# csiro-robotics/syropod_highlevel_controller

Measured on AMD Instinct MI355X. Metric: control-cycles/sec (all legs IK-solved), higher is better.
Workload: dtype f64

## Files before the change

syropod_highlevel_controller_amd/csrc/shc_cycle_kernel.hpp:

```cpp
#pragma once

#include "shc_cycle.hpp"
#include "shc_cycle_launch.hpp"

#include <hip/hip_runtime.h>

namespace shc {

#ifndef SHC_WAVES_PER_SIMD
#define SHC_WAVES_PER_SIMD 2
#endif
#ifndef SHC_ROT_WAVES_PER_SIMD
#define SHC_ROT_WAVES_PER_SIMD 1
#endif
#ifndef SHC_TERRAIN_WAVES_PER_SIMD
#define SHC_TERRAIN_WAVES_PER_SIMD 2
#endif

struct LegPlanes {
  double2 *base;
  int64_t ns;
  uint32_t slot;
  typedef double v2d __attribute__((ext_vector_type(2)));
  __device__ __forceinline__ double2 load(int plane) const { return (base + plane * ns)[slot]; }
// ... 442 lines not shown
        const double fn = norm(in.force());
        const double defined = ld_agent_f64(sp2 + 1);
        if (fn > A.touchdown_threshold && defined == 0.0) {
          Chain<NJ> ch;
          fk_chain<NJ>(C.leg[leg], s.q, ch);
          const V3 tipnow = tip_robot_frame(C.leg[leg], ch.pe);
          if (live) sp[0] = tipnow.x, sp[1] = tipnow.y, sp2[0] = tipnow.z, sp2[1] = 1.0;
        } else if (fn < A.liftoff_threshold) {
          if (live) sp2[1] = 0.0;
        }
      }
    }
    cycle<L, NJ, F>(s, out, C, rb, pk, g, leg, st.legd, ns, slot, dirty, manual_live, touchdown_detection, ext, nullptr, in, publish_previous,
                    (F & F_ROUGH) != 0 ? st.span : nullptr);
    {
      typedef unsigned v4u __attribute__((ext_vector_type(4)));
      double flat[2 * NJ];
#pragma unroll
      for (int i = 0; i < NJ; ++i) flat[FD::Q + i] = s.q[i], flat[FD::QD + i] = s.qd[i];
      const unsigned soff = oslot * out_slot_bytes;
      if (live) {
#pragma unroll
        for (int p = 0; p < NJ; ++p) {
          const u64 a = u64(__double_as_longlong(flat[2 * p])), b = u64(__double_as_longlong(flat[2 * p + 1]));
          const v4u w = {unsigned(a), unsigned(a >> 32), unsigned(b), unsigned(b >> 32)};
          __builtin_amdgcn_raw_buffer_store_b128(w, out_rsrc, unsigned((int64_t(p) * ns + slot) * 16), soff, 16 );
        }
      }
    }
    ++c;
    oslot = oslot + 1 == unsigned(A.depth) ? 0 : oslot + 1;
    gate = uni64(gate_next_v);
    hdr_valid = next_valid;
    if (next_valid) h0 = uni64(n0v), h1 = uni64(n1v);
  }
  if constexpr (!batch) {
    asm volatile("s_waitcnt vmcnt(0)" ::: "memory");
    if (lane == 0) st_agent(A.progress + wave, u64(c));
  }
  held.cycles = c;
}

template <int L, int NJ>
__device__ __forceinline__ void carry_leg_inputs(const ResidentArgs &A, const DevState &st, const ResidentHeld &held, const int64_t ns, const uint32_t slot, const int leg) {
  using FD = Fields<NJ>;
  constexpr int RPW = 64 / L;
  double2 *planes = reinterpret_cast<double2 *>(st.legd);
  const LegInRing<NJ> in = leg_inputs_in_force<L, NJ>(A, st.legd, held.src_force, held.src_effort, ns, slot, int64_t(slot / 64) * RPW + (slot % 64) / L, leg,
                                                      A.batch_cycles ? int64_t(A.batch_cycles) - 1 : 0);
  if (held.src_force != -1) {
    const V3 f = in.force();
    planes[(FD::FORCE_IN / 2) * ns + slot] = double2{f.x, f.y};
    planes[(FD::FORCE_IN / 2 + 1) * ns + slot] = double2{f.z, 0.0};
  }
  if (held.src_effort != -1) {
    double ef[NJ];
    in.effort(ef);
#pragma unroll
    for (int p = 0; p < FD::NJE / 2; ++p) planes[(FD::EFFORT_IN / 2 + p) * ns + slot] = double2{ef[2 * p], 2 * p + 1 < NJ ? ef[2 * p + 1] : 0.0};
  }
}

template <int L, int NJ, unsigned F>
__device__ __forceinline__ void resident_epilogue(const ResidentArgs &A, const DevState &st, const uint32_t slot, const int lane, const bool live,
                                                  const double *tile, const int32_t *tile_i, double *gtile, int32_t *gtile_i, const ResidentHeld &held) {
  using R = RobotFields;
  using FD = Fields<NJ>;
  constexpr int RPW = 64 / L;
  const int64_t ns = st.n_slots;
  store_rob_fields<RPW, R::VIN, R::CORE_END>(tile, gtile, lane);
  if (held.seen & (1u << RG_IMU)) {
    store_rob_fields<RPW, R::GYRO, R::IMU_END>(tile, gtile, lane);
    store_rob_fields<RPW, R::IMUQ, R::IMUQ_END>(tile, gtile, lane);
  }
  if ((held.seen & (1u << RG_RESET)) && lane < RPW) gtile_i[R::I_RESET_MODE * RPW + lane] = tile_i[R::I_RESET_MODE * RPW + lane];
  if (live) carry_leg_inputs<L, NJ>(A, st, held, ns, slot, int(slot % 64) % L);
  if (lane == 0 && A.batch_cycles == 0) {
    if (held.fault) __hip_atomic_fetch_or(&A.ctl->fault, 1ull, __ATOMIC_RELAXED, __HIP_MEMORY_SCOPE_AGENT);
    __hip_atomic_fetch_add(&A.ctl->exited, 1ull, __ATOMIC_RELAXED, __HIP_MEMORY_SCOPE_AGENT);
  }
}

enum : int { PART_BOTH = 0, PART_GATE = 1, PART_DONE = 2 };
template <int PART>
__device__ __forceinline__ void resident_relay(const ResidentArgs &A) {
  const int lane = threadIdx.x & 63;
  const unsigned max_cycles = A.max_cycles;
  unsigned db = 0, sp = max_cycles, idle_stop = 0xffffffffu;
  u64 reason = RESIDENT_EXIT_MAX, last_reason = 0, last_gate = ~0ull, last_done = 0, iter = 0;
  u64 t_last = wall_clock64(), t_all_done = 0;
  for (;;) {
    const u64 now = wall_clock64();
    const u64 exited_v = ld_agent(&A.ctl->exited);
    const u64 gate_v = PART == PART_DONE ? ld_agent(&A.ctl->gate) : 0;
    const u64 done_v = PART != PART_DONE ? ld_agent(&A.ctl->pad[1]) : 0;
    u64 pv[8];
    if (PART != PART_GATE) {
#pragma unroll
      for (int j = 0; j < 8; ++j) pv[j] = j * 64 + lane < A.n_waves ? ld_agent(A.progress + j * 64 + lane) : ~0ull;
    }
    if (PART != PART_DONE) {
      const u64 hd_v = ld_sys(&A.host->doorbell), hs_v = ld_sys(&A.host->stop);
      const u64 rec_v = lane < 2 ? ld_sys(&A.host->records[size_t(db & (kResidentHeaders - 1)) * 2 + lane]) : 0;
      const u64 hd = uni64(hd_v), hs = uni64(hs_v);
      unsigned want_db = hd > max_cycles ? max_cycles : unsigned(hd);
      if (want_db < db) want_db = db;
      if (want_db == db && db < max_cycles) {
        const u64 tag = u64(db) + 1;
        const bool word_ok = lane == 0 ? rec_v == tag : (lane == 1 ? (rec_v >> 48) == (tag & 0xffffull) : true);
        if (__all(word_ok)) {
          const u64 w1 = uni64(__shfl(rec_v, 1, 64));
          if (lane == 0) {
            u64 *hp = reinterpret_cast<u64 *>(A.headers + (db & (kResidentHeaders - 1)));
            st_agent(hp + 1, (w1 & 0x7fffull) | u64(kResidentDirect) | (w1 & 0x30000ull));
            st_agent(hp, tag);
          }
          asm volatile("s_waitcnt vmcnt(0)" ::: "memory");
          want_db = db + 1;
        }
      }
      if (want_db != db || uni64(done_v) < u64(db)) t_last = now;
      else if (idle_stop == 0xffffffffu && now - t_last > A.idle_ticks) idle_stop = db;
      unsigned want_sp = max_cycles;
      u64 why = RESIDENT_EXIT_MAX;
      if (hs <= max_cycles) want_sp = unsigned(hs), why = RESIDENT_EXIT_STOP;
      if (idle_stop < want_sp) want_sp = idle_stop, why = RESIDENT_EXIT_IDLE;
      if (want_sp < db) want_sp = db;
      if (want_db > want_sp) want_db = want_sp;
      db = want_db, sp = want_sp, reason = why;
      if (reason != last_reason) {
        if (lane == 0) st_agent(&A.ctl->pad[0], reason);
        last_reason = reason;
      }
      const u64 gate = (u64(sp) << 32) | db;
      if (gate != last_gate) {
        if (lane == 0) st_agent(&A.ctl->gate, gate);
        last_gate = gate;
      }
    }
    const u64 exited = uni64(exited_v);
    bool leave = exited == u64(A.n_waves);
    if (PART != PART_GATE) {
      if (PART == PART_DONE) sp = unsigned(uni64(gate_v) >> 32);
      u64 m = ~0ull;
#pragma unroll
      for (int j = 0; j < 8; ++j) m = pv[j] < m ? pv[j] : m;
      for (int64_t base = 512; base < A.n_waves; base += 512) {
        u64 v[8];
#pragma unroll
        for (int j = 0; j < 8; ++j) {
          const int64_t w = base + j * 64 + lane;
          v[j] = w < A.n_waves ? ld_agent(A.progress + w) : ~0ull;
        }
#pragma unroll
        for (int j = 0; j < 8; ++j) m = v[j] < m ? v[j] : m;
      }
#pragma unroll
      for (int off = 32; off > 0; off >>= 1) {
        const u64 o = __shfl_xor(m, off, 64);
        m = o < m ? o : m;
      }
      m = uni64(m);
      if (m != last_done) {
        if (lane == 0) {
          st_sys(&A.host->done, m);
          st_agent(&A.ctl->pad[1], m);
        }
        last_done = m;
      }
      bool gave_up = false;
      if (!leave && m >= sp) {
        if (t_all_done == 0) t_all_done = now;
        else if (now - t_all_done > 5000 * A.ticks_per_ms) leave = gave_up = true;
      }
      if (leave) {
        const u64 fault = uni64(ld_agent(&A.ctl->fault));
        const u64 why = uni64(ld_agent(&A.ctl->pad[0]));
        if (lane == 0) {
          st_sys(&A.host->fault, fault);
          st_sys(&A.host->done, m);
          st_agent(&A.ctl->pad[1], m);
          asm volatile("s_waitcnt vmcnt(0)" ::: "memory");
          st_agent(&A.ctl->pad[2], 1ull);
          st_sys(&A.host->exited, (fault || gave_up) ? u64(RESIDENT_EXIT_FAULT) : why);
        }
      }
      if ((++iter & 1023) == 0 && lane == 0) st_sys(&A.host->heartbeat, iter);
    }
    if (leave) break;
    __builtin_amdgcn_s_sleep(1);
  }
}

template <int L, int NJ, unsigned F, bool RES, int HALF = ROLE_ALL, bool BATCH = false>
__device__ __forceinline__ void cycle_wave(const DevState &st, const SharedConsts<L, NJ> *gc, int n_cycles, unsigned rt_flags, const int64_t wave,
                                           const ResidentArgs *ra) {
  static_assert(HALF == ROLE_ALL || (!RES && (F & (F_DYN | F_TERRAIN | F_MLEGS | F_AUTO)) == 0), "half-step launches: feature-exact kernels without auto posing / terrain paths");
  using R = RobotFields;
  using FT = Feat<F>;
  constexpr int RPW = 64 / L;
  __shared__ SharedConsts<L, NJ> C;
  extern __shared__ double wave_lds[];
  constexpr int kWaveDoubles = R::COUNT * RPW + PK_COUNT * 64 + (R::I_COUNT * RPW + 1) / 2;
  SHC_TICK(0);
  const bool manual_live = (rt_flags & RT_MANUAL_LIVE) != 0;
  const bool touchdown_detection = (rt_flags & RT_TOUCHDOWN) != 0;
  const int lane = threadIdx.x & 63;
  const int wib = threadIdx.x >> 6;
  const int64_t rob0 = wave * RPW;
  const int64_t left = st.n_robots - rob0;
  const int robots_here = left < RPW ? (left < 0 ? 0 : int(left)) : RPW;
  int grp = lane / L;
  const int leg = lane - grp * L;
  const bool live = grp < robots_here;
  if (grp >= robots_here) grp = robots_here > 0 ? robots_here - 1 : 0;
  const uint32_t slot = uint32_t(wave * 64 + grp * L + leg);
  double *const my_lds = wave_lds + wib * kWaveDoubles;
  Park pk{my_lds + R::COUNT * RPW, lane};
  LegRegs<NJ> s;
  const CycleParams &GP = gc->P;
  double *tile = my_lds;
  int32_t *tile_i = reinterpret_cast<int32_t *>(my_lds + R::COUNT * RPW + PK_COUNT * 64);
  double *gtile = st.robd + wave * (R::COUNT * RPW);
  int32_t *gtile_i = st.robi + wave * (R::I_COUNT * RPW);
  LegLoad<NJ> ll;
  double th[NJ];
  const bool any_robot = robots_here > 0;
  double2 hand[4] = {double2{0.0, 0.0}, double2{0.0, 0.0}, double2{0.0, 0.0}, double2{0.0, 0.0}};
  double hpose[7] = {0.0, 0.0, 0.0, 1.0, 0.0, 0.0, 0.0};
  double2 qpl[(NJ + 1) / 2];
  int word_back = 0;
  if (any_robot) {
#pragma unroll
    for (int k = 0; k < NJ; ++k) th[k] = gc->leg[leg].link_th[k];
    load_leg_issue<NJ, F, HALF>(ll, st, GP, slot);
    if constexpr (HALF == ROLE_FRONT) {
#pragma unroll
      for (int p = 0; p < (NJ + 1) / 2; ++p) qpl[p] = reinterpret_cast<const double2 *>(st.legd)[p * st.n_slots + slot];
    }
    if constexpr (HALF == ROLE_BACK) {
      word_back = st.legi[slot];
      using FDh = Fields<NJ>;
      static_assert(FDh::TIP % 2 == 0 && FDh::CUR_DIR == FDh::ORG_DIR + 3 && FDh::ORG_DIR % 2 == 0, "plane layout of the walker tip / tip direction");
      const double2 *planes = reinterpret_cast<const double2 *>(st.legd);
      hand[0] = planes[(FDh::TIP / 2) * st.n_slots + slot];
      hand[1] = planes[(FDh::TIP / 2 + 1) * st.n_slots + slot];
      hand[2] = planes[(FDh::ORG_DIR / 2 + 1) * st.n_slots + slot];
      hand[3] = planes[(FDh::ORG_DIR / 2 + 2) * st.n_slots + slot];
#pragma unroll
      for (int k = 0; k < 7; ++k) hpose[k] = gtile[(R::CPOSE + k) * RPW + grp];
    }
  }
  using SC = SharedConsts<L, NJ>;
  static_assert(sizeof(SC) % 16 == 0 && (offsetof(SC, P) + offsetof(CycleParams, ap_start)) % 16 == 0, "const block is copied in 16-byte words");
  constexpr int n16_all = sizeof(SC) / 16;
  constexpr int n16_core = (offsetof(SC, P) + offsetof(CycleParams, ap_start)) / 16;
  const int n16 = FT::autop(GP) ? n16_all : n16_core;
  constexpr int citers = (n16_all + 63) / 64;
  double2 creg[citers];
  {
    const double2 *src = reinterpret_cast<const double2 *>(gc);
    const int nt = blockDim.x;
#pragma unroll
    for (int it = 0; it < citers; ++it) {
      int i = it * nt + threadIdx.x;
      creg[it] = i < n16 ? src[i] : double2{0.0, 0.0};
    }
  }
  double t_core[(R::CORE_END * RPW + 63) / 64], t_man[((R::MANUAL_END - R::MPOSE) * RPW + 63) / 64],
      t_imu[((R::IMU_END - R::ABSE) * RPW + 63) / 64], t_imuq[((R::IMUQ_END - R::IMUQ) * RPW + 63) / 64],
      t_aprev[((R::APREV_END - R::APREV) * RPW + 63) / 64], t_align[((R::COUNT - R::TALIGN) * RPW + 63) / 64], t_odom[((R::ODOM_END - R::ODOM) * RPW + 63) / 64],
      t_cpose[((R::CPOSE_END - R::CPOSE) * RPW + 63) / 64], t_incl[((R::INCL_END - R::INCL) * RPW + 63) / 64];
  const bool skip_marked = (F & F_MLEGS) != 0 && (rt_flags & RT_SKIP_MARKED) != 0 && (rt_flags & RT_MANUAL_LEGS) != 0;
  const bool pose_marked = (F & F_MLEGS) != 0 && (rt_flags & RT_POSE_MARKED) != 0 && (rt_flags & RT_MANUAL_LEGS) != 0;
// ... 274 lines not shown
  if (POSE_SPLIT && walker && lane == 0) X.pose_done[pair] = 0;
  __syncthreads();
  const CycleParams &P = C.P;
  Group<L> g{grp * L};
  RobTile<RPW> rb{tile, tile_i, grp};
  LegOut out;
  out.poser_tip = out.model_tip = out.adm_delta = V3{0, 0, 0};
  s.tipx = V3{1, 0, 0};
  if (active && !walker) {
#pragma unroll
    for (int k = 0; k < NJ; ++k) sincos_joint(C.leg[leg].link_th[k] + s.q[k], &s.sn[k], &s.cs[k]);
    if (FT::adm(P) || LegRegs<NJ>::kKeepJacobian) {
      Chain<NJ> ch;
      chain_from_sincos<NJ>(C.leg[leg], s.sn, s.cs, ch);
      if (LegRegs<NJ>::kKeepJacobian) {
        jacobian_columns<NJ>(ch, s.lin);
        s.pe = ch.pe;
      }
      if (FT::adm(P)) s.tipx = base_rotate(C.leg[leg], ch.xe);
    }
    s.word = 0;
  }
  unsigned dirty = 0;
  ResidentHeld held;
  const int swing_c_count_u = uni(P.swing_c_count);
  const auto publish_for_pose = [&](unsigned cycle, bool planes) {
    if (planes) {
      const V3 pp = rb.get3(R::PLANE_PREV), pn = rb.get3(R::PNORM_PREV);
#pragma unroll
      for (int par = 0; par < 2; ++par) {
        double *mb = &X.mailbox[pair][par][0][lane];
        mb[7 * 64] = pp.x, mb[8 * 64] = pp.y, mb[9 * 64] = pp.z, mb[10 * 64] = pn.x, mb[11 * 64] = pn.y, mb[12 * 64] = pn.z;
      }
    }
    X.pose_c[pair][cycle & 1][lane] = walk_plane_control_candidate<L, NJ>(s.word, C, P, swing_c_count_u);
  };
  if (POSE_SPLIT && walker && active) publish_for_pose(0, true);
  const int64_t ns = st.n_slots;
  const unsigned out_slot_bytes = unsigned(NJ * ns * 16);
  const __amdgpu_buffer_rsrc_t out_rsrc = __builtin_amdgcn_make_buffer_rsrc(A.out, 0, int(unsigned(A.depth) * out_slot_bytes), 0x00020000);
  const u64 emergency_ticks = 4 * A.idle_ticks + 2000 * A.ticks_per_ms;
  unsigned k = 0, c_front = 0, c_back = 0, oslot = 0;
  bool prev_real = false;
  u64 prev_h0 = 0, prev_h1 = 0;
  u64 gate_pref = leader ? ld_agent(&A.ctl->gate) : 0;
  u64 bubble_since = 0;
  FrontToBack fb{V3{1, 0, 0}, false, LS_WALKING};
  fb.uf = load_uni_flags(C.P);
  OdomCache odom_cache;
  Pose owpp_cache = pose_identity();
  if (POSE_SPLIT && active && !walker) owpp_cache = rb.getpose(R::OWPP);
  constexpr bool ODOM_REGS = NJ <= 3;
  constexpr bool ODOM_WALKER = NJ > 3 || (F & (F_ADM | F_IMU | F_INCL | F_AUTO | F_DYN)) != 0;
  double odom[4] = {0.0, 0.0, 1.0, 0.0};
  if (ODOM_REGS && FT::odom(P) && active && walker == ODOM_WALKER) {
#pragma unroll
    for (int i = 0; i < 4; ++i) odom[i] = rb.get(R::ODOM + i);
  }
#ifdef SHC_RES2_TIMING
  long long tm_busy = 0, tm_total0 = __builtin_readcyclecounter(), tm_real = 0;
#ifndef SHC_RES2_BUSY_ONLY
  if (threadIdx.x < 64) shc_acc_lds[threadIdx.x] = 0;
#endif
#endif
#ifdef SHC_RES2_TIMING
#define SHC_R2_ITER_BEGIN() const long long tm0 = __builtin_readcyclecounter(); SHC_TICK(19)
#ifndef SHC_RES2_BUSY_ONLY
#define SHC_R2_PHASES(THREAD, ...)                                                                                                  \
  if (kind == IT_REAL && prev_real && blockIdx.x == 1 && threadIdx.x == (THREAD)) {       \
    const int base = ((THREAD) >> 7) * 32;                                                                                         \
    const int order[] = {__VA_ARGS__};                                                                                             \
    for (int i = 1; i < int(sizeof(order) / sizeof(int)); ++i) shc_acc_lds[base + order[i]] += shc_ticks_lds[base + order[i]] - shc_ticks_lds[base + order[i - 1]]; \
  }
#else
#define SHC_R2_PHASES(THREAD, ...)
#endif
#define SHC_R2_ITER_END(THREAD, ...)                                                         \
  if (kind == IT_REAL && prev_real) tm_busy += __builtin_readcyclecounter() - tm0, ++tm_real; \
  SHC_R2_PHASES(THREAD, __VA_ARGS__)
#else
#define SHC_R2_ITER_BEGIN() do {} while (0)
#define SHC_R2_ITER_END(THREAD, ...) do {} while (0)
#endif
  LegInRing<NJ> in_at;
  int in_src_force = -1000, in_src_effort = -1000;
  if (walker) {
    for (;;) {
      SHC_R2_ITER_BEGIN();
      const int kind = __builtin_amdgcn_readfirstlane(int(X.ctrl[k & 3][0]));
      const u64 h0 = uni64(X.ctrl[k & 3][1]), h1 = uni64(X.ctrl[k & 3][2]);
      SHC_TICK(20);
      if (kind == IT_REAL && active) {
        resident_take_inputs<RPW, POSE_SPLIT ? ROBOT_VEL : ROBOT_ALL, false>(A, c_front, h0, h1, wave, lane, tile, tile_i, dirty, held, st.n_robots);
        SHC_TICK(21);
        const PoseWait<RPW> pose_wait{&X.pose_done[pair], c_front + 1, A.ticks_per_ms, &held.fault};
        cycle_front<L, NJ, F, false, LegInRing<NJ>, false, !POSE_SPLIT>(s, out, C, rb, pk, g, leg, st.legd, ns, slot, dirty, manual_live, false, nullptr, nullptr,
                                                                        LegInRing<NJ>{}, fb, nullptr, pose_wait);
#ifdef SHC_ABLATE
        if (!(P.debug_skip & 65536))
#endif
        if (POSE_SPLIT) publish_for_pose(c_front + 1, fb.plane_prev_changed);
        SHC_TICK(29);
        double *mb = &X.mailbox[pair][c_front & 1][0][lane];
        mb[0] = out.poser_tip.x, mb[64] = out.poser_tip.y, mb[128] = out.poser_tip.z;
        if constexpr (ODOM_WALKER) {
          if (FT::odom(P) && __any(fb.odom_run)) {
            if (fb.odom_run) {
              if constexpr (ODOM_REGS) odometry_advance(odom[0], odom[1], odom[2], odom[3], P, fb.odom_vel.x, fb.odom_vel.y, fb.odom_vel.z, &odom_cache);
              else odometry_step(rb, P, fb.odom_vel.x, fb.odom_vel.y, fb.odom_vel.z, &odom_cache);
            }
          }
        } else if (FT::odom(P)) {
          mb[192] = fb.odom_vel.x, mb[256] = fb.odom_vel.y, mb[320] = fb.odom_vel.z, mb[384] = fb.odom_run ? 1.0 : 0.0;
        }
        SHC_TICK(22);
      }
      SHC_TICK(23);
      if (kind == IT_EXIT) break;
      SHC_R2_ITER_END(0, 19, 20, 21, 2, 3, 4, 5, 6, 7, 16, 8, 17, 15, 29, 22, 23);
      if (kind == IT_REAL) ++c_front;
      prev_real = kind == IT_REAL;
      __syncthreads();
      ++k;
    }
  } else {
    for (;;) {
      SHC_R2_ITER_BEGIN();
      const int kind = __builtin_amdgcn_readfirstlane(int(X.ctrl[k & 3][0]));
      const u64 h0 = uni64(X.ctrl[k & 3][1]), h1 = uni64(X.ctrl[k & 3][2]);
      SHC_TICK(29);
      int nk = IT_EXIT;
      u64 nh0v = 0, nh1v = 0;
      if (leader && kind != IT_EXIT) {
        u64 gate;
        if (kind == IT_BUBBLE) {
          __builtin_amdgcn_s_sleep(2);
          gate = uni64(ld_agent(&A.ctl->gate));
        } else {
          gate = uni64(gate_pref);
        }
        const unsigned db = unsigned(gate), sp = unsigned(gate >> 32);
        const unsigned cn = c_front + (kind == IT_REAL ? 1u : 0u);
        nk = cn >= sp ? IT_EXIT : (cn < db ? IT_REAL : IT_BUBBLE);
        if (nk == IT_BUBBLE) {
          const u64 now = wall_clock64();
          if (bubble_since == 0) bubble_since = now;
          else if (now - bubble_since > emergency_ticks) nk = IT_EXIT, held.fault = true;
        } else {
          bubble_since = 0;
        }
        if (nk == IT_REAL) {
          const u64 *hp = reinterpret_cast<const u64 *>(A.headers + (cn & (kResidentHeaders - 1)));
          nh0v = ld_agent(hp);
          nh1v = ld_agent(hp + 1);
        }
        if (kind == IT_BUBBLE) gate_pref = gate;
        else gate_pref = ld_agent(&A.ctl->gate);
      }
      if (active) {
        SHC_TICK(24);
        if constexpr (POSE_SPLIT) if (kind == IT_REAL) {
          resident_take_inputs<RPW, ROBOT_POSE, false>(A, c_front, h0, h1, wave, lane, tile, tile_i, dirty, held, st.n_robots);
          SHC_TICK(30);
          double pose_c = -1.0;
#pragma unroll
          for (int j = 0; j < L; ++j) {
            const double cj = X.pose_c[pair][c_front & 1][g.base + j];
            pose_c = cj >= 0.0 ? cj : pose_c;
          }
          int lw[L] = {};
          const double *mb = &X.mailbox[pair][c_front & 1][0][lane];
          const V3 plane_prev{mb[7 * 64], mb[8 * 64], mb[9 * 64]}, pnorm_prev{mb[10 * 64], mb[11 * 64], mb[12 * 64]};
          int rword_unused = 0;
          Pose ap = pose_identity(), la = pose_identity();
#ifdef SHC_ABLATE
          if (!(P.debug_skip & 2048))
#endif
          (void)cycle_pose<L, NJ, F, true>(s, C, P, C.leg[leg], rb, g, leg, lw, rword_unused, 0, dirty, manual_live, ap, la, plane_prev, pnorm_prev, fb.uf.swing_c_count, 0,
                                           &owpp_cache, &pose_c);
          __builtin_amdgcn_fence(__ATOMIC_RELEASE, "workgroup");
          __builtin_amdgcn_wave_barrier();
          if (lane == 0) *const_cast<volatile unsigned *>(&X.pose_done[pair]) = c_front + 1;
        }
        SHC_TICK(25);
        if (prev_real) {
          resident_take_inputs<RPW, ROBOT_NONE, true>(A, c_back, prev_h0, prev_h1, wave, lane, tile, tile_i, dirty, held, st.n_robots);
          if (held.src_force != in_src_force || held.src_effort != in_src_effort) {
            in_at = leg_inputs_in_force<L, NJ>(A, st.legd, held.src_force, held.src_effort, ns, slot, wave * RPW + grp, leg);
            in_src_force = held.src_force, in_src_effort = held.src_effort;
          }
          LegInRing<NJ> in = in_at;
          if (FT::tipf(P)) in.prefetch_effort();
          SHC_TICK(31);
          const double *mb = &X.mailbox[pair][c_back & 1][0][lane];
          out.poser_tip = V3{mb[0], mb[64], mb[128]};
          if constexpr (!ODOM_WALKER) if (FT::odom(P)) {
            const V3 ov{mb[192], mb[256], mb[320]};
            if (__any(mb[384] != 0.0)) {
              if (mb[384] != 0.0) {
                if constexpr (ODOM_REGS) odometry_advance(odom[0], odom[1], odom[2], odom[3], P, ov.x, ov.y, ov.z, &odom_cache);
                else odometry_step(rb, P, ov.x, ov.y, ov.z, &odom_cache);
              }
            }
          }
          out.adm_delta = V3{0, 0, 0};
          if (FT::adm(P)) cycle_admittance<NJ>(s, out, P, in);
          s.word = 0;
          SHC_TICK(26);
          cycle_back<L, NJ, F>(s, out, C, leg, st.legd, ns, slot, nullptr, in, fb);
          SHC_TICK(27);
          asm volatile("s_waitcnt vmcnt(0)" ::: "memory");
          if (lane == 0) st_agent(A.progress + wave, u64(c_back));
          SHC_TICK(13);
          {
            typedef unsigned v4u __attribute__((ext_vector_type(4)));
            double flat[2 * NJ];
#pragma unroll
            for (int i = 0; i < NJ; ++i) flat[FD::Q + i] = s.q[i], flat[FD::QD + i] = s.qd[i];
            const unsigned soff = oslot * out_slot_bytes;
#ifdef SHC_ABLATE
            if (!(P.debug_skip & 4096))
#endif
            if (live) {
#pragma unroll
              for (int p = 0; p < NJ; ++p) {
                const u64 a = u64(__double_as_longlong(flat[2 * p])), b = u64(__double_as_longlong(flat[2 * p + 1]));
                const v4u w = {unsigned(a), unsigned(a >> 32), unsigned(b), unsigned(b >> 32)};
                __builtin_amdgcn_raw_buffer_store_b128(w, out_rsrc, unsigned((int64_t(p) * ns + slot) * 16), soff, 16 );
              }
            }
          }
          ++c_back;
          oslot = oslot + 1 == unsigned(A.depth) ? 0 : oslot + 1;
          SHC_TICK(28);
        }
        if (kind != IT_REAL) {
          asm volatile("s_waitcnt vmcnt(0)" ::: "memory");
          if (lane == 0) st_agent(A.progress + wave, u64(c_back));
        }
      }
      if (leader && kind != IT_EXIT && lane == 0) {
        X.ctrl[(k + 1) & 3][0] = u64(nk);
        X.ctrl[(k + 1) & 3][1] = nh0v;
        X.ctrl[(k + 1) & 3][2] = nh1v;
      }
      SHC_TICK(14);
      if (kind == IT_EXIT) break;
      SHC_R2_ITER_END(128, 19, 29, 24, 30, 25, 31, 26, 9, 10, 11, 12, 27, 13, 28, 14);
      if (kind == IT_REAL) ++c_front;
      prev_real = kind == IT_REAL;
      prev_h0 = h0, prev_h1 = h1;
      __syncthreads();
      ++k;
    }
  }
#undef SHC_R2_ITER_BEGIN
#undef SHC_R2_ITER_END
#undef SHC_R2_PHASES
#ifdef SHC_RES2_TIMING
  if (blockIdx.x == 1 && lane == 0 && pair == 0) {
    unsigned long long *dbg = reinterpret_cast<unsigned long long *>(A.ctl) + 8 + (walker ? 0 : 4);
    dbg[0] = tm_busy, dbg[1] = tm_real, dbg[2] = __builtin_readcyclecounter() - tm_total0, dbg[3] = k;
#ifndef SHC_RES2_BUSY_ONLY
    if (walker) {
      for (int i = 0; i < 32; ++i) dbg[8 + i] = (unsigned long long)shc_acc_lds[i];
    } else {
      for (int i = 0; i < 32; ++i) dbg[36 + i] = (unsigned long long)shc_acc_lds[32 + i];
    }
#endif
  }
#endif
  if (active && ODOM_REGS && FT::odom(P) && walker == ODOM_WALKER) {
#pragma unroll
    for (int i = 0; i < 4; ++i) rb.put(R::ODOM + i, odom[i]);
  }
  if (active) {
    if (walker) {
      X.stiff[pair][lane] = s.stiff;
    } else {
      X.ikfail[pair][lane] = s.word & LW_IKFAIL;
      if (POSE_SPLIT) {
        unsigned d = 0;
#pragma unroll
        for (unsigned b = 1; b <= DIRTY_LAST; b <<= 1)
          if (__any((dirty & b) != 0)) d |= b;
        if (lane == 0) X.model_dirty[pair] = d, X.model_seen[pair] = held.seen;
      }
      if (lane == 0) X.model_fault[pair] = held.fault ? 1u : 0u;
    }
  }
  __syncthreads();
  if (!active) return;
  if (walker) {
    if (POSE_SPLIT) dirty |= X.model_dirty[pair], held.seen |= X.model_seen[pair];
    if (X.model_fault[pair]) held.fault = true;
    if (c_front > 0) s.word = (s.word & ~LW_IKFAIL) | X.ikfail[pair][lane];
    {
      unsigned d = 0;
#pragma unroll
      for (unsigned b = 1; b <= DIRTY_LAST; b <<= 1)
        if (__any((dirty & b) != 0)) d |= b;
      dirty = d;
    }
    if (live) store_leg<NJ, F, ROLE_FRONT>(s, out, pk, st, P, slot, dirty);
    __builtin_amdgcn_wave_barrier();
    store_rob_fields<RPW, 0, R::PLANE>(tile, gtile, lane);
    if (dirty & DIRTY_WALK_PLANE) store_rob_fields<RPW, R::PLANE, R::VIN>(tile, gtile, lane);
    if (FT::manual(P) && manual_live && (dirty & DIRTY_MANUAL)) store_rob_fields<RPW, R::MPOSE, R::MANUAL_END>(tile, gtile, lane);
    if (FT::imu(P)) store_rob_fields<RPW, R::ABSE, R::GYRO>(tile, gtile, lane);
    if (FT::incl(P) && FT::autop(P)) store_rob_fields<RPW, R::APREV, R::APREV_END>(tile, gtile, lane);
    store_rob_fields<RPW, R::CPOSE, R::CPOSE_END>(tile, gtile, lane);
    if (FT::odom(P)) store_rob_fields<RPW, R::ODOM, R::ODOM_END>(tile, gtile, lane);
    if (lane < (R::I_POSE_PHASE + 1) * RPW) gtile_i[lane] = tile_i[lane];
    store_rob_fields<RPW, R::VIN, R::CORE_END>(tile, gtile, lane);
    if (held.seen & (1u << RG_IMU)) {
      store_rob_fields<RPW, R::GYRO, R::IMU_END>(tile, gtile, lane);
      store_rob_fields<RPW, R::IMUQ, R::IMUQ_END>(tile, gtile, lane);
    }
    if ((held.seen & (1u << RG_RESET)) && lane < RPW) gtile_i[R::I_RESET_MODE * RPW + lane] = tile_i[R::I_RESET_MODE * RPW + lane];
    if (lane == 0) {
      if (held.fault) __hip_atomic_fetch_or(&A.ctl->fault, 1ull, __ATOMIC_RELAXED, __HIP_MEMORY_SCOPE_AGENT);
      __hip_atomic_fetch_add(&A.ctl->exited, 1ull, __ATOMIC_RELAXED, __HIP_MEMORY_SCOPE_AGENT);
    }
  } else {
    s.stiff = X.stiff[pair][lane];
    if (live) {
      store_leg<NJ, F, ROLE_BACK>(s, out, pk, st, P, slot, 0);
      carry_leg_inputs<L, NJ>(A, st, held, ns, slot, leg);
    }
  }
}

}
```

syropod_highlevel_controller_amd/csrc/shc_resident.hpp:

```cpp

struct Resident {
  bool active = false;
  int depth = 0;
  ResidentArgs args{};
  ResidentHost *host = nullptr;
  ResidentHost *host_dev = nullptr;
  ResidentCtl *ctl = nullptr;
  unsigned long long *progress = nullptr;
  ResidentHeader *headers = nullptr;
  double *rin = nullptr, *force = nullptr, *effort = nullptr, *out = nullptr, *stage = nullptr;
  int32_t *rini = nullptr;
  size_t stage_bytes = 0;
  static constexpr int kPinSlots = 4;
  unsigned *post_blocks_done = nullptr;
  char *pin = nullptr, *pin_dev = nullptr;
  hipEvent_t pin_ev[kPinSlots] = {};
  unsigned long long pin_uses = 0;
  hipStream_t in_stream = nullptr;
  hipStream_t loop_stream = nullptr;
  hipEvent_t loop_ev = nullptr;
  unsigned long long published = 0;
  unsigned long long posted = 0;
  unsigned long long posts[RG_COUNT] = {};
  std::vector<unsigned long long> post_cycle[RG_COUNT];
// ... 519 lines not shown
}

extern "C" int shc_engine_resident_get_joint_state_async(shc_engine *e, int64_t cycle, double *q, double *qd, int timeout_ms) {
  int rc = resident_require(e, true);
  if (rc != SHC_OK) return rc;
  Resident *r = e->res;
  if ((rc = resident_alive(r)) != SHC_OK) return rc;
  if (cycle < 0 || (unsigned long long)cycle >= r->max_cycles) return fail(SHC_ERR_INVALID_ARG, "resident mode: no such cycle (max_cycles)");
  if (r->published > (unsigned long long)cycle + r->depth)
    return fail(SHC_ERR_INVALID_ARG, "resident mode: that cycle's outputs may have been overwritten (ring_depth newer cycles were published)");
  HIP_TRY(hipSetDevice(e->device));
  const unsigned long long ticks = (unsigned long long)(timeout_ms > 0 ? timeout_ms : 5000) * r->wall_khz;
  resident_wait_done_kernel<<<dim3(1), dim3(1), 0, e->stream>>>(r->ctl, r->host_dev, (unsigned long long)cycle + 1, ticks);
  HIP_TRY(hipGetLastError());
  const double *slot = r->out + size_t(cycle % r->depth) * size_t(e->NJ) * e->n_slots * 2;
  const int64_t threads = e->n * e->L;
  for (int which = 0; which < 2; ++which) {
    double *dst = which ? qd : q;
    if (!dst) continue;
    gather_leg_kernel<<<dim3((unsigned)((threads + 63) / 64)), dim3(64), 0, e->stream>>>(dst, slot, e->n_slots, e->n, e->L, e->NJ,
                                                                                         which ? LEG_FIELD(e, QD) : LEG_FIELD(e, Q));
    HIP_TRY(hipGetLastError());
  }
  return SHC_OK;
}

extern "C" int shc_engine_resident_status(shc_engine *e, int64_t *published, int64_t *completed, int32_t *running) {
  int rc = resident_require(e, false);
  if (rc != SHC_OK) return rc;
  Resident *r = e->res;
  const bool active = r && r->active;
  if (published) *published = active ? int64_t(r->published) : 0;
  if (completed) *completed = active ? int64_t(host_load(&r->host->done)) : 0;
  if (running) *running = active && host_load(&r->host->exited) == 0 ? 1 : 0;
  return SHC_OK;
}

extern "C" int shc_engine_resident_end(shc_engine *e, int64_t *cycles_run) {
  int rc = resident_require(e, true);
  if (rc != SHC_OK) return rc;
  Resident *r = e->res;
  HIP_TRY(hipSetDevice(e->device));
  HIP_TRY(hipStreamSynchronize(r->in_stream));
  const int direct_rc = resident_wait_direct_installed(r);
  const std::string direct_msg = direct_rc != SHC_OK ? std::string(shc_last_error()) : std::string();
  if (direct_rc == SHC_OK) host_store(&r->host->doorbell, r->published);
  host_store(&r->host->stop, direct_rc == SHC_OK ? r->published : 0ull);
  const bool answered = spin_until([&] { return host_load(&r->host->exited) != 0; }, r->poisoned ? 5.0 : 30.0);
  if (!answered) {
    r->poisoned = true;
    return fail(SHC_ERR_TIMEOUT, "resident mode: the device loop did not answer the stop request in time; the engine stays in resident mode - call "
                                 "shc_engine_resident_end again");
  }
  hipError_t err = hipStreamSynchronize(r->loop_stream);
  if (err == hipSuccess) err = hipStreamSynchronize(e->stream);
  r->active = false;
  r->poisoned = false;
#ifdef SHC_RES2_TIMING
  if (err == hipSuccess) {
    ResidentCtl c;
    (void)hipMemcpy(&c, r->ctl, sizeof c, hipMemcpyDeviceToHost);
    for (int w = 0; w < 2; ++w)
      fprintf(stderr, "[res2 timing] %s: %.0f clocks busy per steady REAL iteration (%llu of them), loop %llu clocks, %llu iterations\n", w ? "model " : "walker",
              c.dbg[4 * w + 1] ? double(c.dbg[4 * w]) / double(c.dbg[4 * w + 1]) : 0.0, c.dbg[4 * w + 1], c.dbg[4 * w + 2], c.dbg[4 * w + 3]);
#ifndef SHC_RES2_BUSY_ONLY
    const int order[] = {20, 21, 2, 3, 4, 5, 6, 7, 16, 8, 17, 15, 29, 22, 23};
    const char *wname[] = {"control words (LDS) read", "inputs of the cycle taken", "cycle_front entry", "robot word / command read, stop predicates", "(pose elsewhere)", "getLimit",
                           "velocity shaping", "walk state machine", "stepper (stride, Bezier, tip)", "tip rotation / iteratePhase / planes / leg word", "wait for the pose flag",
                           "pose read + updateStance", "control input for the next pose published", "mailbox written", "to the barrier"};
    const double its = c.dbg[1] ? double(c.dbg[1]) : 1.0;
    fprintf(stderr, "[res2 timing] walker of pair 0, mean clocks per phase:\n");
    for (int i = 0; i < int(sizeof(order) / sizeof(int)); ++i) fprintf(stderr, "[res2 timing]   walker t%-2d %-58s %7.0f\n", order[i], wname[i], double(c.dbg[8 + order[i]]) / its);
    const int morder[] = {29, 24, 30, 25, 31, 26, 9, 10, 11, 12, 27, 13, 28, 14};
    const char *mname[] = {"control words (LDS) read", "leader: gate, what the next iteration is, header prefetch issued", "pose inputs of the cycle taken",
                           "updateCurrentPose of the walker's cycle + flag", "leg inputs in force, joint efforts prefetched", "mailbox read, odometry, admittance",
                           "cycle_back entry (desired tip)", "IK step + joint update", "sin / cos, chain, Jacobian", "model tip, tip force", "cycle_back exit",
                           "wait for the previous stores + progress word", "output-ring stores issued", "control words written (leader: waits for its loads)"};
    const double mits = c.dbg[5] ? double(c.dbg[5]) : 1.0;
    fprintf(stderr, "[res2 timing] model wavefront of pair 0 (the leader), mean clocks per phase:\n");
    for (int i = 0; i < int(sizeof(morder) / sizeof(int)); ++i) fprintf(stderr, "[res2 timing]   model  t%-2d %-58s %7.0f\n", morder[i], mname[i], double(c.dbg[40 + morder[i]]) / mits);
#endif
  }
#endif
  const unsigned long long reason = host_load(&r->host->exited), done = host_load(&r->host->done);
  if (cycles_run) *cycles_run = int64_t(done);
  if (r->groups_posted & (1u << RG_FORCE)) e->rt_flags |= RT_TOUCHDOWN;
  if (err != hipSuccess) return fail(SHC_ERR_HIP, std::string("hipStreamSynchronize: ") + hipGetErrorString(err));
  if (direct_rc != SHC_OK) return fail(direct_rc, direct_msg + " (the loop was stopped after " + std::to_string(done) + " cycles)");
  if (reason == RESIDENT_EXIT_FAULT || host_load(&r->host->fault) != 0)
    return fail(SHC_ERR_HIP, "resident mode: a wavefront gave up waiting for the relay; restore the engine from a snapshot");
  if (host_load(&r->host->late_reads) != 0)
    return fail(SHC_ERR_TIMEOUT, "resident mode: a stream-ordered read (shc_engine_resident_get_joint_state_async) gave up waiting for its cycle");
  if (!((reason == RESIDENT_EXIT_STOP || reason == RESIDENT_EXIT_MAX) && done == r->published))
    return fail(SHC_ERR_TIMEOUT, std::string("resident mode: the device loop had stopped by itself (") +
                                     (reason == RESIDENT_EXIT_IDLE ? "idle timeout" : reason == RESIDENT_EXIT_MAX ? "max_cycles" : "unknown") + ") after " +
                                     std::to_string(done) + " of " + std::to_string(r->published) + " published cycles");
  return SHC_OK;
}

static int step_k_out_ring(shc_engine *e, int K) {
  const size_t need = size_t(K) * size_t(e->NJ) * size_t(e->n_slots) * 16;
  if (e->k_out && e->k_out_bytes >= need) return SHC_OK;
  if (e->k_out) {
    const int rc = join_side(e);
    if (rc != SHC_OK) return rc;
    HIP_TRY(hipStreamSynchronize(e->stream));
    (void)hipFree(e->k_out);
    e->k_out = nullptr, e->k_out_bytes = 0;
  }
  HIP_TRY(hipMalloc(reinterpret_cast<void **>(&e->k_out), need));
  e->k_out_bytes = need;
  return SHC_OK;
}

__global__ void copy_joint_planes_kernel(double2 *dst, const double2 *src, int64_t count);
static int step_k_serial(shc_engine *e, int K, const shc_cycle_inputs *in) {
  const int64_t n = e->n, slot = int64_t(e->NJ) * e->n_slots;
  for (int k = 0; k < K; ++k) {
    int rc = SHC_OK;
    if (in && in->linear_xy) rc = shc_engine_set_velocity(e, in->linear_xy + k * n * 2, in->angular + k * n, 1);
    if (rc == SHC_OK && in && in->imu_orientation_wxyz) rc = shc_engine_set_imu(e, in->imu_orientation_wxyz + k * n * 4, in->imu_angular_velocity + k * n * 3, 1);
    if (rc == SHC_OK && in && in->tip_force) rc = shc_engine_set_tip_force(e, in->tip_force + k * n * e->L * 3, 1);
    if (rc == SHC_OK && in && in->joint_effort) rc = shc_engine_set_joint_effort(e, in->joint_effort + k * n * e->L * e->NJ, 1);
    if (rc == SHC_OK) rc = shc_engine_step(e, 1);
    if (rc == SHC_OK) rc = join_side(e);
    if (rc != SHC_OK) return rc;
    copy_joint_planes_kernel<<<dim3((unsigned)((slot + 255) / 256)), dim3(256), 0, e->stream>>>(reinterpret_cast<double2 *>(e->k_out) + k * slot,
                                                                                              reinterpret_cast<const double2 *>(e->st.legd), slot);
    HIP_TRY(hipGetLastError());
  }
  e->k_out_cycles = K;
  return SHC_OK;
}

extern "C" int shc_engine_step_k(shc_engine *e, int n_cycles, const shc_cycle_inputs *in) {
  SHC_ENTER(e);
  if (n_cycles < 1 || n_cycles > 4096) return fail(SHC_ERR_INVALID_ARG, "shc_engine_step_k: 1 .. 4096 cycles per launch");
  if (e->starting_up) return fail(SHC_ERR_UNSUPPORTED, "shc_engine_step_k starts from a running engine (finish the start-up first)");
  unsigned mask = 0;
  if (in) {
    if (!in->on_device) return fail(SHC_ERR_INVALID_ARG, "shc_engine_step_k: the K-deep input arrays are device arrays (on_device = 1)");
    if ((in->linear_xy == nullptr) != (in->angular == nullptr)) return fail(SHC_ERR_INVALID_ARG, "linear_xy and angular are given together");
    if ((in->imu_orientation_wxyz == nullptr) != (in->imu_angular_velocity == nullptr)) return fail(SHC_ERR_INVALID_ARG, "the two IMU arrays are given together");
    if (in->pose_translation_velocity || in->pose_rotation_velocity || in->pose_reset_mode)
      return fail(SHC_ERR_UNSUPPORTED, "shc_engine_step_k carries velocity, IMU, tip force and joint effort; give pose inputs / reset modes with their setters before the call (held for the K cycles)");
    if (in->linear_xy) mask |= 1u << RG_VEL;
    if (in->imu_orientation_wxyz) mask |= 1u << RG_IMU;
    if (in->tip_force) mask |= 1u << RG_FORCE;
    if (in->joint_effort) mask |= 1u << RG_EFFORT;
  }
  HIP_TRY(hipSetDevice(e->device));
  const bool split = e->n_waves >= kSplitWaves && !(e->features & SHC_FEAT_SINGLE_STREAM);
  if (!split || ((mask & (1u << RG_EFFORT)) && !(e->rt_flags & RT_EFFORT_LIVE))) {
    const int rc = join_side(e);
    if (rc != SHC_OK) return rc;
  }
  if (mask & (1u << RG_EFFORT)) {
    const int rc = effort_live(e);
    if (rc != SHC_OK) return rc;
  }
  ResidentFit fit;
  {
    const int rc = resident_fit(e, fit);
    if (rc != SHC_OK) return rc;
  }
  if (size_t(e->NJ) * e->n_slots * 16 * size_t(n_cycles) >= (size_t(1) << 31))
// ... 80 lines not shown
```

Baseline: 1.573 billion.

## Pipeline relay doorbell polling with multiple in-flight samples and drop gate sleep

The gate-side relay now keeps several doorbell/control samples in flight in a small ring, processing one sample while the next loads are outstanding, and no longer sleeps between polls. Each sample's host and control words are gathered by lane and read with readlane. The done-side progress scan uses wider unrolled batches, and model wavefronts reuse a prefetched gate value when a bubble is followed by another non-real iteration. The aim is to cut host-doorbell-to-device latency in the resident loop, at the cost of acting on slightly stale samples and busier polling of system memory.

```diff
diff --git a/syropod_highlevel_controller_amd/csrc/shc_cycle_kernel.hpp b/syropod_highlevel_controller_amd/csrc/shc_cycle_kernel.hpp
--- a/syropod_highlevel_controller_amd/csrc/shc_cycle_kernel.hpp
+++ b/syropod_highlevel_controller_amd/csrc/shc_cycle_kernel.hpp
@@ -548,114 +548,162 @@
 }
 
 enum : int { PART_BOTH = 0, PART_GATE = 1, PART_DONE = 2 };
+#ifndef SHC_RELAY_DEPTH
+#define SHC_RELAY_DEPTH 4
+#endif
+static_assert(SHC_RELAY_DEPTH >= 1 && SHC_RELAY_DEPTH <= 4, "doorbell samples in flight");
+#ifndef SHC_DONE_ROUND
+#define SHC_DONE_ROUND 16
+#endif
+struct RelaySample {
+  u64 host_v;
+  u64 ctl_v;
+  unsigned db;
+};
+static_assert(offsetof(ResidentCtl, dbg) == 64 && offsetof(ResidentHost, doorbell) == 0 && offsetof(ResidentHost, stop) == 8 && offsetof(ResidentCtl, gate) == 0 && offsetof(ResidentCtl, exited) == 8 && offsetof(ResidentCtl, pad) == 24, "the samples address these words by lane");
+__device__ __forceinline__ RelaySample relay_sample_issue(const ResidentArgs &A, const unsigned db, const int lane) {
+  const int l4 = lane & 3;
+  const u64 *hp = l4 < 2 ? reinterpret_cast<const u64 *>(A.host) + l4 : &A.host->records[size_t(db & (kResidentHeaders - 1)) * 2 + (l4 & 1)];
+  return RelaySample{ld_sys(hp), ld_agent(reinterpret_cast<const u64 *>(A.ctl) + (lane & 7)), db};
+}
+__device__ __forceinline__ u64 lane64(const u64 v, const int l) {
+  return (u64(unsigned(__builtin_amdgcn_readlane(int(unsigned(v >> 32)), l))) << 32) | unsigned(__builtin_amdgcn_readlane(int(unsigned(v)), l));
+}
 template <int PART>
 __device__ __forceinline__ void resident_relay(const ResidentArgs &A) {
+  constexpr int D = PART == PART_GATE ? SHC_RELAY_DEPTH : 1;
   const int lane = threadIdx.x & 63;
   const unsigned max_cycles = A.max_cycles;
   unsigned db = 0, sp = max_cycles, idle_stop = 0xffffffffu;
   u64 reason = RESIDENT_EXIT_MAX, last_reason = 0, last_gate = ~0ull, last_done = 0, iter = 0;
   u64 t_last = wall_clock64(), t_all_done = 0;
+#ifdef SHC_RELAY_TIMING
+  const u64 tm_begin = wall_clock64();
+#endif
+  RelaySample ring[D];
+  if (PART != PART_DONE) {
+#pragma unroll
+    for (int i = 0; i < D; ++i) ring[i] = relay_sample_issue(A, db, lane);
+  }
+  bool leave = false;
   for (;;) {
-    const u64 now = wall_clock64();
-    const u64 exited_v = ld_agent(&A.ctl->exited);
-    const u64 gate_v = PART == PART_DONE ? ld_agent(&A.ctl->gate) : 0;
-    const u64 done_v = PART != PART_DONE ? ld_agent(&A.ctl->pad[1]) : 0;
-    u64 pv[8];
-    if (PART != PART_GATE) {
-#pragma unroll
-      for (int j = 0; j < 8; ++j) pv[j] = j * 64 + lane < A.n_waves ? ld_agent(A.progress + j * 64 + lane) : ~0ull;
-    }
-    if (PART != PART_DONE) {
-      const u64 hd_v = ld_sys(&A.host->doorbell), hs_v = ld_sys(&A.host->stop);
-      const u64 rec_v = lane < 2 ? ld_sys(&A.host->records[size_t(db & (kResidentHeaders - 1)) * 2 + lane]) : 0;
-      const u64 hd = uni64(hd_v), hs = uni64(hs_v);
-      unsigned want_db = hd > max_cycles ? max_cycles : unsigned(hd);
-      if (want_db < db) want_db = db;
-      if (want_db == db && db < max_cycles) {
-        const u64 tag = u64(db) + 1;
-        const bool word_ok = lane == 0 ? rec_v == tag : (lane == 1 ? (rec_v >> 48) == (tag & 0xffffull) : true);
-        if (__all(word_ok)) {
-          const u64 w1 = uni64(__shfl(rec_v, 1, 64));
+#pragma unroll
+    for (int i = 0; i < D; ++i) {
+      const u64 now = wall_clock64();
+      u64 exited = 0;
+      bool posted = false;
+      if (PART != PART_DONE) {
+        const RelaySample s = ring[i];
+        const u64 hd = lane64(s.host_v, 0), hs = lane64(s.host_v, 1);
+        const u64 done_v = lane64(s.ctl_v, 4);
+        exited = lane64(s.ctl_v, 1);
+        unsigned want_db = hd > max_cycles ? max_cycles : unsigned(hd);
+        if (want_db < db) want_db = db;
+        if (want_db == db && db < max_cycles && s.db == db) {
+          const u64 tag = u64(db) + 1;
+          const bool word_ok = lane == 2 ? s.host_v == tag : (lane == 3 ? (s.host_v >> 48) == (tag & 0xffffull) : true);
+          if (__all(word_ok)) {
+            const u64 w1 = lane64(s.host_v, 3);
+            if (lane == 0) {
+              u64 *hp = reinterpret_cast<u64 *>(A.headers + (db & (kResidentHeaders - 1)));
+              st_agent(hp + 1, (w1 & 0x7fffull) | u64(kResidentDirect) | (w1 & 0x30000ull));
+              st_agent(hp, tag);
+            }
+            posted = true;
+            want_db = db + 1;
+          }
+        }
+        if (want_db != db || done_v < u64(db)) t_last = now;
+        else if (idle_stop == 0xffffffffu && now - t_last > A.idle_ticks) idle_stop = db;
+        unsigned want_sp = max_cycles;
+        u64 why = RESIDENT_EXIT_MAX;
+        if (hs <= max_cycles) want_sp = unsigned(hs), why = RESIDENT_EXIT_STOP;
+        if (idle_stop < want_sp) want_sp = idle_stop, why = RESIDENT_EXIT_IDLE;
+        if (want_sp < db) want_sp = db;
+        if (want_db > want_sp) want_db = want_sp;
+        db = want_db, sp = want_sp, reason = why;
+      }
+      u64 ctl_now = 0, pv[SHC_DONE_ROUND];
+      if (PART == PART_DONE) ctl_now = lane < 2 ? ld_agent(reinterpret_cast<const u64 *>(A.ctl) + lane) : 0;
+      if (PART != PART_GATE) {
+#pragma unroll
+        for (int j = 0; j < SHC_DONE_ROUND; ++j) pv[j] = j * 64 + lane < A.n_waves ? ld_agent(A.progress + j * 64 + lane) : ~0ull;
+      }
+      if (PART != PART_DONE) {
+        ring[i] = relay_sample_issue(A, db, lane);
+        if (posted) asm volatile("s_waitcnt vmcnt(0)" ::: "memory");
+        if (reason != last_reason) {
+          if (lane == 0) st_agent(&A.ctl->pad[0], reason);
+          last_reason = reason;
+        }
+        const u64 gate = (u64(sp) << 32) | db;
+        if (gate != last_gate) {
+          if (lane == 0) st_agent(&A.ctl->gate, gate);
+          last_gate = gate;
+        }
+      }
+      if (PART == PART_DONE) exited = lane64(ctl_now, 1);
+      leave |= exited == u64(A.n_waves);
+      if (PART != PART_GATE) {
+        if (PART == PART_DONE) sp = unsigned(lane64(ctl_now, 0) >> 32);
+        u64 m = ~0ull;
+#pragma unroll
+        for (int j = 0; j < SHC_DONE_ROUND; ++j) m = pv[j] < m ? pv[j] : m;
+        for (int64_t base = 64 * SHC_DONE_ROUND; base < A.n_waves; base += 64 * SHC_DONE_ROUND) {
+          u64 v[SHC_DONE_ROUND];
+#pragma unroll
+          for (int j = 0; j < SHC_DONE_ROUND; ++j) {
+            const int64_t w = base + j * 64 + lane;
+            v[j] = w < A.n_waves ? ld_agent(A.progress + w) : ~0ull;
+          }
+#pragma unroll
+          for (int j = 0; j < SHC_DONE_ROUND; ++j) m = v[j] < m ? v[j] : m;
+        }
+#pragma unroll
+        for (int off = 32; off > 0; off >>= 1) {
+          const u64 o = __shfl_xor(m, off, 64);
+          m = o < m ? o : m;
+        }
+        m = uni64(m);
+        if (m != last_done) {
           if (lane == 0) {
-            u64 *hp = reinterpret_cast<u64 *>(A.headers + (db & (kResidentHeaders - 1)));
-            st_agent(hp + 1, (w1 & 0x7fffull) | u64(kResidentDirect) | (w1 & 0x30000ull));
-            st_agent(hp, tag);
+            st_sys(&A.host->done, m);
+            st_agent(&A.ctl->pad[1], m);
           }
-          asm volatile("s_waitcnt vmcnt(0)" ::: "memory");
-          want_db = db + 1;
-        }
-      }
-      if (want_db != db || uni64(done_v) < u64(db)) t_last = now;
-      else if (idle_stop == 0xffffffffu && now - t_last > A.idle_ticks) idle_stop = db;
-      unsigned want_sp = max_cycles;
-      u64 why = RESIDENT_EXIT_MAX;
-      if (hs <= max_cycles) want_sp = unsigned(hs), why = RESIDENT_EXIT_STOP;
-      if (idle_stop < want_sp) want_sp = idle_stop, why = RESIDENT_EXIT_IDLE;
-      if (want_sp < db) want_sp = db;
-      if (want_db > want_sp) want_db = want_sp;
-      db = want_db, sp = want_sp, reason = why;
-      if (reason != last_reason) {
-        if (lane == 0) st_agent(&A.ctl->pad[0], reason);
-        last_reason = reason;
-      }
-      const u64 gate = (u64(sp) << 32) | db;
-      if (gate != last_gate) {
-        if (lane == 0) st_agent(&A.ctl->gate, gate);
-        last_gate = gate;
-      }
-    }
-    const u64 exited = uni64(exited_v);
-    bool leave = exited == u64(A.n_waves);
-    if (PART != PART_GATE) {
-      if (PART == PART_DONE) sp = unsigned(uni64(gate_v) >> 32);
-      u64 m = ~0ull;
-#pragma unroll
-      for (int j = 0; j < 8; ++j) m = pv[j] < m ? pv[j] : m;
-      for (int64_t base = 512; base < A.n_waves; base += 512) {
-        u64 v[8];
-#pragma unroll
-        for (int j = 0; j < 8; ++j) {
-          const int64_t w = base + j * 64 + lane;
-          v[j] = w < A.n_waves ? ld_agent(A.progress + w) : ~0ull;
-        }
-#pragma unroll
-        for (int j = 0; j < 8; ++j) m = v[j] < m ? v[j] : m;
-      }
-#pragma unroll
-      for (int off = 32; off > 0; off >>= 1) {
-        const u64 o = __shfl_xor(m, off, 64);
-        m = o < m ? o : m;
-      }
-      m = uni64(m);
-      if (m != last_done) {
-        if (lane == 0) {
-          st_sys(&A.host->done, m);
-          st_agent(&A.ctl->pad[1], m);
-        }
-        last_done = m;
-      }
-      bool gave_up = false;
-      if (!leave && m >= sp) {
-        if (t_all_done == 0) t_all_done = now;
-        else if (now - t_all_done > 5000 * A.ticks_per_ms) leave = gave_up = true;
-      }
-      if (leave) {
-        const u64 fault = uni64(ld_agent(&A.ctl->fault));
-        const u64 why = uni64(ld_agent(&A.ctl->pad[0]));
-        if (lane == 0) {
-          st_sys(&A.host->fault, fault);
-          st_sys(&A.host->done, m);
-          st_agent(&A.ctl->pad[1], m);
-          asm volatile("s_waitcnt vmcnt(0)" ::: "memory");
-          st_agent(&A.ctl->pad[2], 1ull);
-          st_sys(&A.host->exited, (fault || gave_up) ? u64(RESIDENT_EXIT_FAULT) : why);
-        }
-      }
-      if ((++iter & 1023) == 0 && lane == 0) st_sys(&A.host->heartbeat, iter);
+          last_done = m;
+        }
+        bool gave_up = false;
+        if (!leave && m >= sp) {
+          if (t_all_done == 0) t_all_done = now;
+          else if (now - t_all_done > 5000 * A.ticks_per_ms) leave = gave_up = true;
+        }
+        if (leave) {
+          const u64 fault = uni64(ld_agent(&A.ctl->fault));
+          const u64 why = uni64(ld_agent(&A.ctl->pad[0]));
+          if (lane == 0) {
+            st_sys(&A.host->fault, fault);
+            st_sys(&A.host->done, m);
+            st_agent(&A.ctl->pad[1], m);
+            asm volatile("s_waitcnt vmcnt(0)" ::: "memory");
+            st_agent(&A.ctl->pad[2], 1ull);
+            st_sys(&A.host->exited, (fault || gave_up) ? u64(RESIDENT_EXIT_FAULT) : why);
+          }
+        }
+        if ((++iter & 1023) == 0 && lane == 0) st_sys(&A.host->heartbeat, iter);
+      }
+#ifdef SHC_RELAY_TIMING
+      if (PART == PART_GATE) ++iter;
+#endif
+      if (PART == PART_DONE) __builtin_amdgcn_s_sleep(1);
     }
     if (leave) break;
-    __builtin_amdgcn_s_sleep(1);
-  }
+  }
+#ifdef SHC_RELAY_TIMING
+  if (lane == 0) {
+    A.ctl->dbg[PART == PART_DONE ? 74 : 72] = iter;
+    A.ctl->dbg[PART == PART_DONE ? 75 : 73] = wall_clock64() - tm_begin;
+  }
+#endif
 }
 
 template <int L, int NJ, unsigned F, bool RES, int HALF = ROLE_ALL, bool BATCH = false>
@@ -1096,6 +1144,9 @@
 #define SHC_R2_ITER_BEGIN() do {} while (0)
 #define SHC_R2_ITER_END(THREAD, ...) do {} while (0)
 #endif
+#ifdef SHC_RELAY_TIMING
+  unsigned long long tm_falls = 0;
+#endif
   LegInRing<NJ> in_at;
   int in_src_force = -1000, in_src_effort = -1000;
   if (walker) {
@@ -1168,7 +1219,11 @@
           nh0v = ld_agent(hp);
           nh1v = ld_agent(hp + 1);
         }
+#ifndef SHC_NO_BURST_HEAD
+        if (kind == IT_BUBBLE && nk != IT_REAL) gate_pref = gate;
+#else
         if (kind == IT_BUBBLE) gate_pref = gate;
+#endif
         else gate_pref = ld_agent(&A.ctl->gate);
       }
       if (active) {
@@ -1260,6 +1315,9 @@
       }
       SHC_TICK(14);
       if (kind == IT_EXIT) break;
+#ifdef SHC_RELAY_TIMING
+      if (leader && blockIdx.x == 1 && kind == IT_BUBBLE && prev_real) ++tm_falls;
+#endif
       SHC_R2_ITER_END(128, 19, 29, 24, 30, 25, 31, 26, 9, 10, 11, 12, 27, 13, 28, 14);
       if (kind == IT_REAL) ++c_front;
       prev_real = kind == IT_REAL;
@@ -1283,6 +1341,9 @@
     }
 #endif
   }
+#endif
+#ifdef SHC_RELAY_TIMING
+  if (leader && blockIdx.x == 1 && lane == 0) A.ctl->dbg[76] = tm_falls;
 #endif
   if (active && ODOM_REGS && FT::odom(P) && walker == ODOM_WALKER) {
 #pragma unroll
diff --git a/syropod_highlevel_controller_amd/csrc/shc_resident.hpp b/syropod_highlevel_controller_amd/csrc/shc_resident.hpp
--- a/syropod_highlevel_controller_amd/csrc/shc_resident.hpp
+++ b/syropod_highlevel_controller_amd/csrc/shc_resident.hpp
@@ -625,6 +625,15 @@
 #endif
   }
 #endif
+#ifdef SHC_RELAY_TIMING
+  if (err == hipSuccess) {
+    ResidentCtl c;
+    (void)hipMemcpy(&c, r->ctl, sizeof c, hipMemcpyDeviceToHost);
+    const double us_per_tick = 1e3 / double(r->args.ticks_per_ms);
+    fprintf(stderr, "[relay timing] gate side: %llu samples, one per %.3f us; done side: %llu scans, one per %.3f us; the pipeline ran dry %llu times\n", c.dbg[72],
+            c.dbg[72] ? double(c.dbg[73]) * us_per_tick / double(c.dbg[72]) : 0.0, c.dbg[74], c.dbg[74] ? double(c.dbg[75]) * us_per_tick / double(c.dbg[74]) : 0.0, c.dbg[76]);
+  }
+#endif
   const unsigned long long reason = host_load(&r->host->exited), done = host_load(&r->host->done);
   if (cycles_run) *cycles_run = int64_t(done);
   if (r->groups_posted & (1u << RG_FORCE)) e->rt_flags |= RT_TOUCHDOWN;
```

Measured after the change: 1.572 billion. No clear change (-0.0%).
